# sharmaabhijith/safe-dreamer

Measured on AMD Instinct MI355X. Metric: imagined latent steps/sec at B16·L64·H15, 1/2/4/8 MI355X; WM-loss Δ vs ref, higher is better.
Workload: dtype f32 (split-bf16 gradient GEMMs); 1 GPU; dmc walker_walk vision 64x64x3, rep_loss=r2dreamer (BASELINE configs[1]), per-GPU B16 L64 H15; config=dmc/cnn, global_batch=16, per_gpu_batch=16, seq_len=64, imag_horizon=15, parallelism=dp1

## Files before the change

### safe-dreamer_amd/csrc/conv.hip

```cpp
#include <stdlib.h>

#include "gemm3_core.h"
#include "gemm6_core.h"
#include "gemm_core.h"
#include "sdhip.h"

extern "C" int sd_colsum(const float* in, float* out, int R, int N, long ld, int accumulate, sd_stream s);
extern "C" int sd_colsum_ws(const float* in, float* out, int R, int N, long ld, int accumulate, float* workspace,
                            sd_stream s);

namespace {
using namespace sdg;

struct Geom {
  const float* in;
  int Nb, Hs, Ws, C;
  int Hg, Wg;
  int kh, kw, pad, ups;
};

SD_DEV bool tap(const Geom& G, int n, int y, int x, int k, long& off) {
  const int t = k / G.C, c = k - t * G.C;
  const int ky = t / G.kw, kx = t - ky * G.kw;
  const int yy = y + ky - G.pad, xx = x + kx - G.pad;
// ... 439 lines not shown
                 : f32x4{0.f, 0.f, 0.f, 0.f};
    }
#pragma unroll
    for (int e = 0; e < NE; ++e) {
      const int i = tid + 256 * e;
      if (i < NEL) {
        const int c4 = i % CI4, pix = i / CI4;
        float h0, h1, h2, h3, m0, m1, m2, m3;
        const u32x2 h{bf16_pair(v[e][0], v[e][1], h0, h1), bf16_pair(v[e][2], v[e][3], h2, h3)};
        const float r0 = v[e][0] - h0, r1 = v[e][1] - h1, r2 = v[e][2] - h2, r3 = v[e][3] - h3;
        const u32x2 m{bf16_pair(r0, r1, m0, m1), bf16_pair(r2, r3, m2, m3)};
        const f32x4 l{r0 - m0, r1 - m1, r2 - m2, r3 - m3};
        __bf16* dst = patch6 + pix * CP + 4 * c4;
        *reinterpret_cast<u32x2*>(dst) = h;
        *reinterpret_cast<u32x2*>(dst + PLANE) = m;
        *reinterpret_cast<bf16x4*>(dst + 2 * PLANE) = __builtin_convertvector(l, bf16x4);
      }
    }
  }
  int pbase[2];
#pragma unroll
  for (int mt = 0; mt < 2; ++mt) {
    const int p = 32 * wave + 16 * mt + l16;
    pbase[mt] = ((p >> LW) * PW + (p & (W - 1))) * CP;
  }
  const __bf16* wl = wsp + (long)l16 * KP + 8 * q;
  bf16x8 b[2][TN][3];
  auto bload = [&](int kc, int s) {
#pragma unroll
    for (int j = 0; j < TN; ++j)
#pragma unroll
      for (int pl = 0; pl < 3; ++pl)
        b[s][j][pl] = *reinterpret_cast<const bf16x8*>(wl + ((long)pl * BN + 16 * j) * KP + 32 * kc);
  };
  f32x4 acc[2][TN];
#pragma unroll
  for (int i = 0; i < 2; ++i)
#pragma unroll
    for (int j = 0; j < TN; ++j) acc[i][j] = f32x4{0.f, 0.f, 0.f, 0.f};
  bload(0, 0);
  __syncthreads();
  auto chunk = [&](int kc, int s) {
    if (kc + 1 < NKC) bload(kc + 1, s ^ 1);
    int k0 = 32 * kc + 8 * q;
    k0 = k0 < K ? k0 : K - 8;
    const int tap = k0 / CI, c0 = k0 - tap * CI, ky = tap / KS, kx = tap - ky * KS;
    const int off = (ky * PW + kx) * CP + c0;
    bf16x8 a[2][3];
#pragma unroll
    for (int mt = 0; mt < 2; ++mt)
#pragma unroll
      for (int pl = 0; pl < 3; ++pl) a[mt][pl] = *reinterpret_cast<const bf16x8*>(patch6 + pl * PLANE + pbase[mt] + off);
#pragma unroll
    for (int mt = 0; mt < 2; ++mt)
#pragma unroll
      for (int j = 0; j < TN; ++j) {
        f32x4 c = acc[mt][j];
        c = __builtin_amdgcn_mfma_f32_16x16x32_bf16(a[mt][2], b[s][j][0], c, 0, 0, 0);
        c = __builtin_amdgcn_mfma_f32_16x16x32_bf16(a[mt][1], b[s][j][1], c, 0, 0, 0);
        c = __builtin_amdgcn_mfma_f32_16x16x32_bf16(a[mt][0], b[s][j][2], c, 0, 0, 0);
        c = __builtin_amdgcn_mfma_f32_16x16x32_bf16(a[mt][1], b[s][j][0], c, 0, 0, 0);
        c = __builtin_amdgcn_mfma_f32_16x16x32_bf16(a[mt][0], b[s][j][1], c, 0, 0, 0);
        acc[mt][j] = __builtin_amdgcn_mfma_f32_16x16x32_bf16(a[mt][0], b[s][j][0], c, 0, 0, 0);
      }
  };
  int kc = 0;
  for (; kc + 2 <= NKC; kc += 2) {
    chunk(kc, 0);
    chunk(kc + 1, 1);
  }
  if (kc < NKC) chunk(kc, 0);
  __syncthreads();
  pool_epilogue<BN, 32>(acc, reinterpret_cast<float*>(patch6), g, G, LW, lhw, bm0, nw, pooled, amax, y, rstd, eps,
                        nchw_flat);
}

template <int BN, int CI, int LW, int KS, int TPW, int MT = 2, int BROW = 40, class NW = const float*>
__global__ __launch_bounds__(512, 1) void conv_fwd6r_direct_pool(GemmArgs g, Geom G, int lhw,
                                                                  const __bf16* __restrict__ wsp, NW nw,
                                                                  float* pooled, uint8_t* amax, float* y, float* rstd,
                                                                  float eps, int nchw_flat) {
  constexpr int NTH = 512, TP = 16 * MT * (NTH / 64);
  constexpr int W = 1 << LW, R = TP / W, PH = R + KS - 1, PW = W + KS - 1, PAD = KS / 2;
  constexpr int NPIX = PH * PW, PLANE = NPIX * CI, K = KS * KS * CI, NKC = (K + 31) / 32, KP = NKC * 32, TN = BN / 16;
  constexpr int CI4 = CI / 4, NEL = PH * PW * CI4, NE = (NEL + NTH - 1) / NTH;
  constexpr int SB = 3 * BN * BROW, NPC = 3 * BN * 4, NPT = (NPC + NTH - 1) / NTH;
  auto poff = [](int pix, int c) { return ((c >> 3) * NPIX + pix) * 8 + (c & 7); };
  static_assert(CI % 8 == 0 && TP % W == 0 && BN % 16 == 0, "geometry");
  static_assert(TP * (BN + 1) * 4 <= 3 * PLANE * 2, "epilogue tile fits the patch area");
  typedef __bf16 bf16x8 __attribute__((ext_vector_type(8)));
  extern __shared__ __attribute__((aligned(16))) __bf16 patch6r[];
  const int tid = threadIdx.x, lane = tid & 63, wave = tid >> 6, l16 = lane & 15, q = lane >> 4;
  const int nwg = gridDim.x, ntiles = g.M / TP;
  const int wg = (nwg & 7) ? blockIdx.x : (blockIdx.x & 7) * (nwg >> 3) + (blockIdx.x >> 3);
  __bf16* bst = patch6r + 3 * PLANE;
  bf16x8 br[NPT];
  auto bload = [&](int kc) {
#pragma unroll
    for (int u = 0; u < NPT; ++u) {
      const int i = tid + NTH * u;
      if (i < NPC) br[u] = *reinterpret_cast<const bf16x8*>(wsp + (long)(i >> 2) * KP + 32 * kc + 8 * (i & 3));
    }
  };
  auto bstore = [&](int st) {
#pragma unroll
    for (int u = 0; u < NPT; ++u) {
      const int i = tid + NTH * u;
      if (i < NPC) *reinterpret_cast<bf16x8*>(bst + st * SB + (i >> 2) * BROW + 8 * (i & 3)) = br[u];
    }
  };
  f32x4 v[NE];
  auto load_patch = [&](int tile) {
    const int bm0 = tile * TP, n = bm0 >> lhw, y0 = (bm0 & ((1 << lhw) - 1)) >> LW;
#pragma unroll
    for (int e = 0; e < NE; ++e) {
      const int i = tid + NTH * e, c4 = i % CI4, pix = i / CI4, pc = pix % PW, pr = pix / PW;
      const int yy = y0 + pr - PAD, xx = pc - PAD;
      v[e] = (i < NEL && tile < ntiles && (unsigned)yy < (unsigned)G.Hs && (unsigned)xx < (unsigned)W)
                 ? *reinterpret_cast<const f32x4*>(G.in + (((long)n * G.Hs + yy) * W + xx) * CI + 4 * c4)
                 : f32x4{0.f, 0.f, 0.f, 0.f};
    }
  };
  auto store_patch = [&]() {
#pragma unroll
    for (int e = 0; e < NE; ++e) {
      const int i = tid + NTH * e;
      if (i < NEL) {
        const int c4 = i % CI4, pix = i / CI4;
        float h0, h1, h2, h3, m0, m1, m2, m3;
        const u32x2 h{bf16_pair(v[e][0], v[e][1], h0, h1), bf16_pair(v[e][2], v[e][3], h2, h3)};
        const float r0 = v[e][0] - h0, r1 = v[e][1] - h1, r2 = v[e][2] - h2, r3 = v[e][3] - h3;
        const u32x2 m{bf16_pair(r0, r1, m0, m1), bf16_pair(r2, r3, m2, m3)};
        const f32x4 l{r0 - m0, r1 - m1, r2 - m2, r3 - m3};
        __bf16* dst = patch6r + poff(pix, 4 * c4);
        *reinterpret_cast<u32x2*>(dst) = h;
        *reinterpret_cast<u32x2*>(dst + PLANE) = m;
        *reinterpret_cast<bf16x4*>(dst + 2 * PLANE) = __builtin_convertvector(l, bf16x4);
      }
    }
  };
  int pbase[MT];
#pragma unroll
  for (int mt = 0; mt < MT; ++mt) {
    const int p = 16 * MT * wave + 16 * mt + l16;
    pbase[mt] = (p >> LW) * PW + (p & (W - 1));
  }
  bload(0);
  load_patch(wg * TPW);
  for (int it = 0; it < TPW; ++it) {
  const int tile = wg * TPW + it;
  if (tile >= ntiles) break;
  if (it > 0) __syncthreads();
  store_patch();
  bstore(0);
  if (NKC > 1) bload(1);
  f32x4 acc[MT][TN];
#pragma unroll
  for (int i = 0; i < MT; ++i)
#pragma unroll
    for (int j = 0; j < TN; ++j) acc[i][j] = f32x4{0.f, 0.f, 0.f, 0.f};
  __syncthreads();
  if (it + 1 < TPW) load_patch(tile + 1);
  for (int kc = 0; kc < NKC; ++kc) {
    const __bf16* bs = bst + (kc & 1) * SB + l16 * BROW + 8 * q;
    bf16x8 b[TN][3];
#pragma unroll
    for (int j = 0; j < TN; ++j)
#pragma unroll
      for (int pl = 0; pl < 3; ++pl) b[j][pl] = *reinterpret_cast<const bf16x8*>(bs + (pl * BN + 16 * j) * BROW);
    int k0 = 32 * kc + 8 * q;
    k0 = k0 < K ? k0 : K - 8;
    const int tap = k0 / CI, c0 = k0 - tap * CI, ky = tap / KS, kx = tap - ky * KS;
    const int toff = ky * PW + kx;
    bf16x8 a[MT][3];
#pragma unroll
    for (int mt = 0; mt < MT; ++mt)
#pragma unroll
      for (int pl = 0; pl < 3; ++pl)
        a[mt][pl] = *reinterpret_cast<const bf16x8*>(patch6r + pl * PLANE + poff(pbase[mt] + toff, c0));
    if (kc + 1 < NKC) bstore((kc + 1) & 1);
    if (kc + 2 < NKC) bload(kc + 2);
#pragma unroll
    for (int mt = 0; mt < MT; ++mt)
#pragma unroll
      for (int j = 0; j < TN; ++j) {
        f32x4 c = acc[mt][j];
        c = __builtin_amdgcn_mfma_f32_16x16x32_bf16(a[mt][2], b[j][0], c, 0, 0, 0);
        c = __builtin_amdgcn_mfma_f32_16x16x32_bf16(a[mt][1], b[j][1], c, 0, 0, 0);
        c = __builtin_amdgcn_mfma_f32_16x16x32_bf16(a[mt][0], b[j][2], c, 0, 0, 0);
        c = __builtin_amdgcn_mfma_f32_16x16x32_bf16(a[mt][1], b[j][0], c, 0, 0, 0);
        c = __builtin_amdgcn_mfma_f32_16x16x32_bf16(a[mt][0], b[j][1], c, 0, 0, 0);
        acc[mt][j] = __builtin_amdgcn_mfma_f32_16x16x32_bf16(a[mt][0], b[j][0], c, 0, 0, 0);
      }
    __syncthreads();
  }
  if (it + 1 < TPW) bload(0);
  pool_epilogue<BN, 16 * MT>(acc, reinterpret_cast<float*>(patch6r), g, G, LW, lhw, tile * TP, nw, pooled, amax, y,
                             rstd, eps, nchw_flat);
  }
}

__global__ __launch_bounds__(256) void split3_weight(const float* __restrict__ w, __bf16* __restrict__ out, int rows,
                                                     int K, int KP) {
  const long i = (long)blockIdx.x * 256 + threadIdx.x;
  if (i >= (long)rows * KP) return;
  const int r = (int)(i / KP), k = (int)(i % KP);
  const float v = k < K ? w[(long)r * K + k] : 0.f;
  const __bf16 a0 = (__bf16)v;
  const float r1 = v - (float)a0;
  const __bf16 a1 = (__bf16)r1;
  const long pl = (long)rows * KP;
  out[i] = a0;
  out[pl + i] = a1;
  out[2 * pl + i] = (__bf16)(r1 - (float)a1);
}

template <int BN, int LW, int KS, int OCC, class NW = const float*>
__global__ __launch_bounds__(256, OCC) void conv_fwd_direct_pool_c4(GemmArgs g, Geom G, int lhw, int TPW,
                                                                    NW nw, float* pooled, uint8_t* amax,
                                                                    float* y, float* rstd, float eps, int nchw_flat) {
  constexpr int BM = 128, WM = 32, TM = WM / 16, TN = BN / 16, W = 1 << LW, R = BM / W;
  constexpr int PH = R + KS - 1, PW = W + KS - 1, PAD = KS / 2, NT = KS * KS;
  constexpr int NQ = PH * PW, NQT = (NQ + 255) / 256;
  float* smem = sd_smem<NQT * 256 * 4 + BM * (BN + 1)>();
  float* patch = smem;
  float* C = smem + NQT * 256 * 4;
  const int nwg = gridDim.x, ntiles = g.M / BM;
  const int wg = (nwg & 7) ? blockIdx.x : (blockIdx.x & 7) * (nwg >> 3) + (blockIdx.x >> 3);
  const int lane = threadIdx.x & 63, wave = threadIdx.x >> 6, l16 = lane & 15, q = lane >> 4;
  float bw[NT][TN];
  {
    const sd_rsrc rb = sd_make_rsrc(g.B, (long)g.N * g.ldb * 4);
#pragma unroll
    for (int t = 0; t < NT; ++t)
#pragma unroll
      for (int j = 0; j < TN; ++j) bw[t][j] = sd_bload1(rb, (uint32_t)(((16 * j + l16) * g.ldb + 4 * t + q) * 4));
  }
  EpiPre<BN> pre;
#pragma unroll
  for (int j = 0; j < TN; ++j) pre.bias[j] = g.bias ? g.bias[16 * j + l16] : 0.f;
#pragma unroll
  for (int k = 0; k < BN / 8; ++k) pre.nw[k] = nw_of(nw)[(threadIdx.x & 7) + 8 * k];
  const sd_rsrc rs = sd_make_rsrc(G.in, (long)G.Nb * G.Hs * G.Ws * 16);
  f32x4 v[NQT];
  auto load_patch = [&](int tile) {
    const int bm0 = tile * BM, n = bm0 >> lhw, y0 = (bm0 & ((1 << lhw) - 1)) >> LW;
#pragma unroll
    for (int u = 0; u < NQT; ++u) {
      const int i = threadIdx.x + 256 * u;
      const int py = i / PW, px = i % PW;
      const int yy = y0 + py - PAD, xx = px - PAD;
      const bool ok = i < NQ && tile < ntiles && (unsigned)yy < (unsigned)G.Hs && (unsigned)xx < (unsigned)W;
      v[u] = sd_bload4(rs, ok ? (uint32_t)(((n * G.Hs + yy) * W + xx) * 16) : SD_OOB);
    }
  };
  int abase[TM];
#pragma unroll
  for (int i = 0; i < TM; ++i) {
    const int p = wave * WM + 16 * i + l16;
    abase[i] = ((p >> LW) * PW + (p & (W - 1))) * 4 + q;
  }
  load_patch(wg * TPW);
  for (int it = 0; it < TPW; ++it) {
    const int tile = wg * TPW + it;
    if (tile >= ntiles) break;
#pragma unroll
    for (int u = 0; u < NQT; ++u) *reinterpret_cast<f32x4*>(patch + 4 * (threadIdx.x + 256 * u)) = v[u];
    __syncthreads();
    if (it + 1 < TPW) load_patch(tile + 1);
    f32x4 acc[TM][TN];
#pragma unroll
    for (int i = 0; i < TM; ++i)
#pragma unroll
      for (int j = 0; j < TN; ++j) acc[i][j] = f32x4{0.f, 0.f, 0.f, 0.f};
#pragma unroll
    for (int t = 0; t < NT; ++t) {
      const int toff = ((t / KS) * PW + t % KS) * 4;
      float a[TM];
#pragma unroll
      for (int i = 0; i < TM; ++i) a[i] = patch[abase[i] + toff];
#pragma unroll
      for (int i = 0; i < TM; ++i)
#pragma unroll
        for (int j = 0; j < TN; ++j)
          acc[i][j] = __builtin_amdgcn_mfma_f32_16x16x4f32(a[i], bw[t][j], acc[i][j], 0, 0, 0);
    }
    __syncthreads();
    pool_epilogue<BN, WM>(acc, C, g, G, LW, lhw, tile * BM, nw, pooled, amax, y, rstd, eps, nchw_flat, &pre);
  }
}


struct DirectW {
  const float* x;
  const float* dy;
  const uint8_t* amax;
  float* ws;
  int Nb, H, W, Ci, Co, kh, kw, pad, R, lw;
  int J, PW, PH, CP, DS, blocks;
};

constexpr int WD_VA = 4, WD_VP = 6;

template <int TM, bool PL>
struct WdF32 {
  const DirectW& d;
  const int tid, nA;
  float* const dyl;
  float* const xp;
  f32x4 ra[WD_VA];
  uint32_t aa[PL ? WD_VA : 1];
  SD_DEV WdF32(const DirectW& d_, float* lds, int tid_)
      : d(d_), tid(tid_), nA(d_.R * d_.W * d_.Co / 4), dyl(lds), xp(lds + d_.R * d_.W * d_.DS) {}
  SD_DEV void init() {
    for (int pix = tid; pix < d.PH * d.PW; pix += 512) {
      xp[pix * d.CP + d.Ci] = 1.f;
      xp[pix * d.CP + d.Ci + 1] = 0.f;
    }
  }
  SD_DEV void fetch_dy(int n, int y0) {
    const float* dsrc = d.dy + ((long)n * d.H + y0) * d.W * d.Co;
#pragma unroll
    for (int v = 0; v < WD_VA; ++v) {
      const int i = tid + 512 * v;
      if constexpr (PL) {
        ra[v] = f32x4{0.f, 0.f, 0.f, 0.f};
        aa[v] = 0xffffffffu;
        if (i < nA / 4) {
          const long pp = (((long)n * (d.H >> 1) + (y0 >> 1)) * (d.W >> 1)) * d.Co + 4 * i;
          ra[v] = *reinterpret_cast<const f32x4*>(d.dy + pp);
          aa[v] = *reinterpret_cast<const uint32_t*>(d.amax + pp);
        }
      } else {
        ra[v] = i < nA ? *reinterpret_cast<const f32x4*>(dsrc + 4 * i) : f32x4{0.f, 0.f, 0.f, 0.f};
      }
    }
  }
  SD_DEV void stage_dy() {
#pragma unroll
    for (int v = 0; v < WD_VA; ++v) {
      const int i = tid + 512 * v;
      if constexpr (PL) {
        if (i < nA / 4) {
          const int e = 4 * i, pl = e / d.Co, c = e - pl * d.Co;
          const int hw = d.W >> 1, pr = pl / hw, pc = pl - pr * hw;
#pragma unroll
          for (int qd = 0; qd < 4; ++qd) {
            const int p = (2 * pr + (qd >> 1)) * d.W + 2 * pc + (qd & 1);
            f32x4 val;
#pragma unroll
            for (int k = 0; k < 4; ++k) val[k] = ((aa[v] >> (8 * k)) & 0xffu) == (uint32_t)qd ? ra[v][k] : 0.f;
            *reinterpret_cast<f32x4*>(dyl + p * d.DS + c) = val;
          }
        }
      } else if (i < nA) {
        const int e = 4 * i, p = e / d.Co, c = e - p * d.Co;
        *reinterpret_cast<f32x4*>(dyl + p * d.DS + c) = ra[v];
      }
    }
  }
  SD_DEV void stage_patch(int pix, int c, const f32x4& v) { *reinterpret_cast<f32x4*>(xp + pix * d.CP + c) = v; }
  template <int NBW, bool WS>
  SD_DEV void contract(f32x4 (&acc)[TM][NBW], const int (&off)[NBW], int P, int wave, int l16, int q) {
    for (int s = WS ? wave : 0; s < P / 4; s += WS ? NW_D : 1) {
      const int p = 4 * s + q, py = p >> d.lw, px = p & (d.W - 1);
      float a[TM];
#pragma unroll
      for (int i = 0; i < TM; ++i) a[i] = dyl[p * d.DS + 16 * i + l16];
      const float* xb = xp + (py * d.PW + px) * d.CP;
      float bv[NBW];
#pragma unroll
      for (int b = 0; b < NBW; ++b) bv[b] = xb[off[b]];
#pragma unroll
      for (int b = 0; b < NBW; ++b)
#pragma unroll
        for (int i = 0; i < TM; ++i) acc[i][b] = __builtin_amdgcn_mfma_f32_16x16x4f32(a[i], bv[b], acc[i][b], 0, 0, 0);
    }
  }
};

SD_DEV uint32_t pack_split(float v) {
  const f32x4 x = {v, 0.f, 0.f, 0.f};
  sdb::bf16x4 hi, lo;
  sdb::split2(x, hi, lo);
  return (uint32_t)__builtin_bit_cast(uint16_t, hi[0]) | ((uint32_t)__builtin_bit_cast(uint16_t, lo[0]) << 16);
}

template <int TM, bool PL>
struct WdBf16x3 {
  typedef uint32_t u32x4 __attribute__((ext_vector_type(4)));
  const DirectW& d;
  const int tid;
  float* const xp;
  __bf16* const dyh;
  __bf16* const dyl;
  int nD, dq4, dc, dih, dsb;
  f32x4 rd[4];
  uint32_t aw[PL ? 4 : 1];
  int qd[PL ? 4 : 1];
  SD_DEV WdBf16x3(const DirectW& d_, float* lds, int tid_)
      : d(d_), tid(tid_), xp(lds), dyh(reinterpret_cast<__bf16*>(lds + d_.PH * d_.PW * d_.CP)),
        dyl(dyh + TM * 16 * d_.DS) {
    for (int e = tid; e < TM * 16 * d.DS; e += 512) {
      dyh[e] = (__bf16)0.f;
      dyl[e] = (__bf16)0.f;
    }
  }
  SD_DEV void init() {
    const int c4 = d.Co / 4, drest = tid / c4;
    nD = c4 * (d.R * d.W / 4);
    dq4 = tid % c4;
    dc = drest % 4, dih = (drest / 4) % 2, dsb = drest / 8;
    for (int pix = tid; pix < d.PH * d.PW; pix += 512) {
      reinterpret_cast<uint32_t*>(xp)[pix * d.CP + d.Ci] = pack_split(1.f);
      reinterpret_cast<uint32_t*>(xp)[pix * d.CP + d.Ci + 1] = 0u;
    }
  }
  SD_DEV void fetch_dy(int n, int y0) {
    [[maybe_unused]] const float* dsrc = d.dy + ((long)n * d.H + y0) * d.W * d.Co;
#pragma unroll
    for (int t = 0; t < 4; ++t) {
      const int px = 32 * dsb + dc + 4 * (4 * dih + t);
      if constexpr (PL) {
        const int yy = y0 + (px >> d.lw), xx = px & (d.W - 1);
        const long pp = (((long)n * (d.H >> 1) + (yy >> 1)) * (d.W >> 1) + (xx >> 1)) * d.Co + 4 * dq4;
        const bool ok = tid < nD;
        rd[t] = ok ? *reinterpret_cast<const f32x4*>(d.dy + pp) : f32x4{0.f, 0.f, 0.f, 0.f};
        aw[t] = ok ? *reinterpret_cast<const uint32_t*>(d.amax + pp) : 0xffffffffu;
        qd[t] = (yy & 1) * 2 + (xx & 1);
      } else {
        rd[t] = tid < nD ? *reinterpret_cast<const f32x4*>(dsrc + (long)px * d.Co + 4 * dq4)
                         : f32x4{0.f, 0.f, 0.f, 0.f};
      }
    }
  }
  SD_DEV void stage_dy() {
    if (tid < nD) {
      const int pos = 32 * dsb + 8 * dc + 4 * dih;
      if constexpr (PL) {
#pragma unroll
        for (int t = 0; t < 4; ++t)
#pragma unroll
          for (int k = 0; k < 4; ++k)
            if (((aw[t] >> (8 * k)) & 0xffu) != (uint32_t)qd[t]) rd[t][k] = 0.f;
      }
#pragma unroll
      for (int jj = 0; jj < 4; ++jj) {
        const f32x4 t = {rd[0][jj], rd[1][jj], rd[2][jj], rd[3][jj]};
        sdb::bf16x4 hi, lo;
        sdb::split2(t, hi, lo);
        const int o = (4 * dq4 + jj) * d.DS + pos;
        *reinterpret_cast<sdb::bf16x4*>(dyh + o) = hi;
        *reinterpret_cast<sdb::bf16x4*>(dyl + o) = lo;
      }
    }
  }
  SD_DEV void stage_patch(int pix, int c, const f32x4& v) {
    sdb::bf16x4 hi, lo;
    sdb::split2(v, hi, lo);
    const uint64_t h = __builtin_bit_cast(uint64_t, hi), l = __builtin_bit_cast(uint64_t, lo);
    u32x4 w;
#pragma unroll
    for (int k = 0; k < 4; ++k) w[k] = (uint32_t)((h >> (16 * k)) & 0xffffu) | ((uint32_t)((l >> (16 * k)) & 0xffffu) << 16);
    *reinterpret_cast<u32x4*>(xp + pix * d.CP + c) = w;
  }
  template <int NBW, bool WS>
  SD_DEV void contract(f32x4 (&acc)[TM][NBW], const int (&off)[NBW], int P, int wave, int l16, int q) {
    for (int s = WS ? wave : 0; s < P / 32; s += WS ? NW_D : 1) {
      sdb::bf16x8 ah[TM], al[TM];
#pragma unroll
      for (int i = 0; i < TM; ++i) {
        const int o = (16 * i + l16) * d.DS + 32 * s + 8 * q;
        ah[i] = *reinterpret_cast<const sdb::bf16x8*>(dyh + o);
        al[i] = *reinterpret_cast<const sdb::bf16x8*>(dyl + o);
      }
      int pb[8];
#pragma unroll
      for (int i = 0; i < 8; ++i) {
        const int p = 32 * s + 4 * i + q, py = p >> d.lw, px = p & (d.W - 1);
        pb[i] = (py * d.PW + px) * d.CP;
      }
#pragma unroll
      for (int b = 0; b < NBW; ++b) {
        const uint32_t* xu = reinterpret_cast<const uint32_t*>(xp);
        uint32_t wv[8];
#pragma unroll
        for (int i = 0; i < 8; ++i) wv[i] = xu[pb[i] + off[b]];
        u32x4 ph, pl;
#pragma unroll
        for (int i = 0; i < 4; ++i) {
          ph[i] = __builtin_amdgcn_perm(wv[2 * i + 1], wv[2 * i], 0x05040100u);
          pl[i] = __builtin_amdgcn_perm(wv[2 * i + 1], wv[2 * i], 0x07060302u);
        }
        const sdb::bf16x8 bh = __builtin_bit_cast(sdb::bf16x8, ph), bl = __builtin_bit_cast(sdb::bf16x8, pl);
#pragma unroll
        for (int i = 0; i < TM; ++i) {
          acc[i][b] = __builtin_amdgcn_mfma_f32_16x16x32_bf16(al[i], bh, acc[i][b], 0, 0, 0);
          acc[i][b] = __builtin_amdgcn_mfma_f32_16x16x32_bf16(ah[i], bl, acc[i][b], 0, 0, 0);
          acc[i][b] = __builtin_amdgcn_mfma_f32_16x16x32_bf16(ah[i], bh, acc[i][b], 0, 0, 0);
        }
      }
    }
  }
};

template <class M, int TM, int NBW, bool WS>
SD_DEV void wgrad_direct_body(const DirectW& d) {
  extern __shared__ __attribute__((aligned(16))) float lds[];
  const int tid = threadIdx.x, lane = tid & 63, wave = tid >> 6;
  const int l16 = lane & 15, q = lane >> 4;
  const int P = d.R * d.W;
  M m(d, lds, tid);
  int off[NBW];
#pragma unroll
  for (int b = 0; b < NBW; ++b) {
    const int j = 16 * (WS ? b : (blockIdx.x * NW_D + wave) * NBW + b) + l16;
    if (j < d.J) {
      const int t = j / d.Ci, ci = j - t * d.Ci, ky = t / d.kw, kx = t - ky * d.kw;
      off[b] = (ky * d.PW + kx) * d.CP + ci;
    } else {
      off[b] = d.Ci + (j == d.J ? 0 : 1);
    }
  }
  f32x4 acc[TM][NBW];
#pragma unroll
  for (int i = 0; i < TM; ++i)
#pragma unroll
    for (int b = 0; b < NBW; ++b) acc[i][b] = f32x4{0.f, 0.f, 0.f, 0.f};
  const int rows_per_img = d.H / d.R, cq = d.Ci / 4, nP = d.PH * d.PW * cq;
  f32x4 rp[WD_VP];
  auto fetch = [&](int rb) {
    const int n = rb / rows_per_img, y0 = (rb - n * rows_per_img) * d.R;
    m.fetch_dy(n, y0);
#pragma unroll
    for (int v = 0; v < WD_VP; ++v) {
      const int i = tid + 512 * v;
      f32x4 x = {0.f, 0.f, 0.f, 0.f};
      if (i < nP) {
        const int pix = i / cq, c = 4 * (i - pix * cq);
        const int py = pix / d.PW, px = pix - py * d.PW;
        const int iy = y0 - d.pad + py, ix = px - d.pad;
        if (iy >= 0 && iy < d.H && ix >= 0 && ix < d.W)
          x = *reinterpret_cast<const f32x4*>(d.x + (((long)n * d.H + iy) * d.W + ix) * d.Ci + c);
      }
      rp[v] = x;
    }
  };
  auto stage = [&]() {
    m.stage_dy();
#pragma unroll
    for (int v = 0; v < WD_VP; ++v) {
      const int i = tid + 512 * v;
      if (i < nP) {
        const int pix = i / cq, c = 4 * (i - pix * cq);
        m.stage_patch(pix, c, rp[v]);
      }
    }
  };
  m.init();
  int rb = blockIdx.y;
  if (rb < d.blocks) fetch(rb);
  for (; rb < d.blocks; rb += gridDim.y) {
    __syncthreads();
    stage();
    __syncthreads();
    if (rb + (int)gridDim.y < d.blocks) fetch(rb + gridDim.y);
    m.template contract<NBW, WS>(acc, off, P, wave, l16, q);
  }
  float* out = d.ws + (long)blockIdx.y * d.Co * (d.J + 1);
  if constexpr (WS) {
#pragma unroll
    for (int b = 0; b < NBW; ++b)
#pragma unroll
      for (int i = 0; i < TM; ++i) {
        __syncthreads();
#pragma unroll
        for (int r = 0; r < 4; ++r) lds[(wave * 4 + r) * 64 + lane] = acc[i][b][r];
        __syncthreads();
        if (tid < 256) {
          const int r = tid >> 6, ln = tid & 63;
          float v = 0.f;
#pragma unroll
          for (int w = 0; w < NW_D; ++w) v += lds[(w * 4 + r) * 64 + ln];
          const int j = 16 * b + (ln & 15), co = 16 * i + 4 * (ln >> 4) + r;
          if (j <= d.J && co < d.Co) out[(long)co * (d.J + 1) + j] = v;
        }
      }
    return;
  }
#pragma unroll
  for (int b = 0; b < NBW; ++b) {
    const int j = 16 * ((blockIdx.x * NW_D + wave) * NBW + b) + l16;
    if (j <= d.J) {
#pragma unroll
      for (int i = 0; i < TM; ++i)
#pragma unroll
        for (int r = 0; r < 4; ++r) {
          const int co = 16 * i + 4 * q + r;
          if (co < d.Co) out[(long)co * (d.J + 1) + j] = acc[i][b][r];
        }
    }
  }
}

template <int TM, int NBW, bool WS, bool PL = false>
__global__ __launch_bounds__(512) void conv_wgrad_direct(DirectW d) {
  wgrad_direct_body<WdF32<TM, PL>, TM, NBW, WS>(d);
}
template <int TM, int NBW, bool WS = false, bool PL = false>
__global__ __launch_bounds__(512) void conv_wgrad3_direct(DirectW d) {
  wgrad_direct_body<WdBf16x3<TM, PL>, TM, NBW, WS>(d);
}


template <class L, int ROWS>
struct KCSplit {
  L& l;
  SD_DEV explicit KCSplit(L& l_) : l(l_) {}
  SD_DEV void load(int k0, int kend) { l.load(k0, kend); }
  SD_DEV void store(__bf16* lds) const {
#pragma unroll
    for (int v = 0; v < L::NV; ++v) {
      const int i = threadIdx.x + v * 256;
      if ((v + 1) * 256 <= ROWS * BK / 4 || i < ROWS * BK / 4)
        sdb::split_store(lds + (i / (BK / 4)) * sdb::LROW + 4 * (i % (BK / 4)), l.st.r[v]);
    }
  }
};

template <int BN>
__global__ __launch_bounds__(256, 2) void conv_dgrad3(GemmArgs g, Geom G, int lw, int lhw) {
  __shared__ int tab[MAX_TAPQ];
  build_taps(tab, G, g.K);
  constexpr int BM = 128;
  const int bm0 = blockIdx.x * BM;
  Im2colRowsB<BM> la0(G, tab, g.M, bm0, lw, lhw);
  DenseKCB<BN> lb0(g.B, g.ldb, g.N, 0);
  KCSplit<Im2colRowsB<BM>, BM> la(la0);
  KCSplit<DenseKCB<BN>, BN> lb(lb0);
  f32x4 acc[2][BN / 16];
  sdb::gemm3_mainloop<BM, BN, 32, BN>(la, lb, 0, g.K, acc);
  epilogue16<BM, BN, 32, BN>(g, acc, bm0, 0, 0, 0);
}

template <int CIN, int NT, int LW, int KS, int NTHR>
__global__ __launch_bounds__(NTHR, 2) void conv_dgrad3_direct(const float* __restrict__ dout,
                                                               const __bf16* __restrict__ wsp, float* __restrict__ din,
                                                               int Nb, int H, int pad) {
  constexpr int MT = 4, TP = 16 * MT * (NTHR / 64);
  constexpr int W = 1 << LW, R = TP / W, PH = R + KS - 1, PW = W + KS - 1, NPIX = PH * PW;
  constexpr int PLANE = NPIX * CIN, K = KS * KS * CIN, NKC = (K + 31) / 32, KP = NKC * 32, NOUT = 16 * NT;
  constexpr int CIN4 = CIN / 4, NEL = PH * PW * CIN4, NE = (NEL + NTHR - 1) / NTHR;
  static_assert(CIN % 8 == 0 && R >= 1 && TP % W == 0, "geometry");
  auto poff = [](int pix, int c) { return ((c >> 3) * NPIX + pix) * 8 + (c & 7); };
  extern __shared__ __attribute__((aligned(16))) __bf16 patch[];
  const int tid = threadIdx.x, lane = tid & 63, wave = tid >> 6, l16 = lane & 15, q = lane >> 4;
  const int rows_per_img = H / R, n = blockIdx.x / rows_per_img, y0 = (blockIdx.x % rows_per_img) * R;
  {
    f32x4 v[NE];
#pragma unroll
    for (int e = 0; e < NE; ++e) {
      const int i = tid + NTHR * e, c4 = i % CIN4, pix = i / CIN4, pc = pix % PW, pr = pix / PW;
      const int y = y0 + pr - pad, x = pc - pad;
      v[e] = (i < NEL && y >= 0 && y < H && x >= 0 && x < W)
                 ? *reinterpret_cast<const f32x4*>(dout + (((long)n * H + y) * W + x) * CIN + 4 * c4)
                 : f32x4{0.f, 0.f, 0.f, 0.f};
    }
#pragma unroll
    for (int e = 0; e < NE; ++e) {
      const int i = tid + NTHR * e;
      if (i < NEL) {
        const int c4 = i % CIN4, pix = i / CIN4;
        sdb::bf16x4 hi, lo;
        sdb::split2(v[e], hi, lo);
        *reinterpret_cast<sdb::bf16x4*>(patch + poff(pix, 4 * c4)) = hi;
        *reinterpret_cast<sdb::bf16x4*>(patch + PLANE + poff(pix, 4 * c4)) = lo;
      }
    }
  }
  int pbase[MT];
#pragma unroll
  for (int mt = 0; mt < MT; ++mt) {
    const int p = 16 * MT * wave + 16 * mt + l16;
    pbase[mt] = (p >> LW) * PW + (p & (W - 1));
  }
  typedef __bf16 bf16x8 __attribute__((ext_vector_type(8)));
  constexpr int BROW = 40, SB = 2 * NOUT * BROW, NPC = 8 * NOUT, NPT = (NPC + NTHR - 1) / NTHR;
  __bf16* bst = patch + 2 * PLANE;
  bf16x8 br[NPT];
  auto bload = [&](int kc) {
#pragma unroll
    for (int u = 0; u < NPT; ++u) {
      const int i = tid + NTHR * u;
      if (i < NPC) br[u] = *reinterpret_cast<const bf16x8*>(wsp + (long)(i >> 2) * KP + 32 * kc + 8 * (i & 3));
    }
  };
  auto bstore = [&](int stage) {
#pragma unroll
    for (int u = 0; u < NPT; ++u) {
      const int i = tid + NTHR * u;
      if (i < NPC) *reinterpret_cast<bf16x8*>(bst + stage * SB + (i >> 2) * BROW + 8 * (i & 3)) = br[u];
    }
  };
  f32x4 acc[MT][NT];
#pragma unroll
  for (int i = 0; i < MT; ++i)
#pragma unroll
    for (int j = 0; j < NT; ++j) acc[i][j] = f32x4{0.f, 0.f, 0.f, 0.f};
  bload(0);
  bstore(0);
  if (NKC > 1) bload(1);
  __syncthreads();
  for (int kc = 0; kc < NKC; ++kc) {
    const __bf16* bs = bst + (kc & 1) * SB + l16 * BROW + 8 * q;
    bf16x8 bh[NT], bl[NT];
#pragma unroll
    for (int j = 0; j < NT; ++j) {
      bh[j] = *reinterpret_cast<const bf16x8*>(bs + 16 * j * BROW);
      bl[j] = *reinterpret_cast<const bf16x8*>(bs + (NOUT + 16 * j) * BROW);
    }
    int k0 = 32 * kc + 8 * q;
    k0 = k0 < K ? k0 : K - 8;
    const int tap = k0 / CIN, c0 = k0 - tap * CIN, ky = tap / KS, kx = tap - ky * KS;
    const int toff = ky * PW + kx;
    bf16x8 ah[MT], al[MT];
#pragma unroll
    for (int mt = 0; mt < MT; ++mt) {
      ah[mt] = *reinterpret_cast<const bf16x8*>(patch + poff(pbase[mt] + toff, c0));
      al[mt] = *reinterpret_cast<const bf16x8*>(patch + PLANE + poff(pbase[mt] + toff, c0));
    }
    if (kc + 1 < NKC) bstore((kc + 1) & 1);
    if (kc + 2 < NKC) bload(kc + 2);
#pragma unroll
    for (int mt = 0; mt < MT; ++mt)
#pragma unroll
      for (int j = 0; j < NT; ++j) {
        acc[mt][j] = __builtin_amdgcn_mfma_f32_16x16x32_bf16(al[mt], bh[j], acc[mt][j], 0, 0, 0);
        acc[mt][j] = __builtin_amdgcn_mfma_f32_16x16x32_bf16(ah[mt], bl[j], acc[mt][j], 0, 0, 0);
        acc[mt][j] = __builtin_amdgcn_mfma_f32_16x16x32_bf16(ah[mt], bh[j], acc[mt][j], 0, 0, 0);
      }
    __syncthreads();
  }
#pragma unroll
  for (int mt = 0; mt < MT; ++mt)
#pragma unroll
    for (int r = 0; r < 4; ++r) {
      const int p = 16 * MT * wave + 16 * mt + 4 * q + r, y = y0 + (p >> LW), x = p & (W - 1);
      float* o = din + (((long)n * H + y) * W + x) * NOUT + l16;
#pragma unroll
      for (int j = 0; j < NT; ++j) o[16 * j] = acc[mt][j][r];
    }
}

__global__ __launch_bounds__(256) void split_weight(const float* __restrict__ w, __bf16* __restrict__ out, int rows,
                                                    int K, int KP) {
  const long i = (long)blockIdx.x * 256 + threadIdx.x;
  if (i >= (long)rows * KP) return;
  const int r = (int)(i / KP), k = (int)(i % KP);
  const float v = k < K ? w[(long)r * K + k] : 0.f;
  const __bf16 hi = (__bf16)v;
  out[i] = hi;
  out[(long)rows * KP + i] = (__bf16)(v - (float)hi);
}

__global__ __launch_bounds__(256) void slab_reduce(const float* __restrict__ ws, int slabs, long n,
                                                   float* __restrict__ out, sd_wgrad_acc acc, int J, int cx) {
  __shared__ float part[4][64];
  const int lane = threadIdx.x & 63, wave = threadIdx.x >> 6;
  const long e = (long)blockIdx.x * 64 + lane;
  float v = 0.f;
  if (e < n) {
    int s = wave;
    for (; s + 12 < slabs; s += 16) {
      const float a0 = ws[(long)s * n + e], a1 = ws[(long)(s + 4) * n + e];
      const float a2 = ws[(long)(s + 8) * n + e], a3 = ws[(long)(s + 12) * n + e];
      v += (a0 + a1) + (a2 + a3);
    }
    for (; s < slabs; s += 4) v += ws[(long)s * n + e];
  }
  part[wave][lane] = v;
  __syncthreads();
  if (wave == 0 && e < n) {
    const float r = (part[0][lane] + part[1][lane]) + (part[2][lane] + part[3][lane]);
    if (!acc.dw) {
      out[e] = r;
    } else {
      const long co = e / (J + 1);
      const int j = (int)(e - co * (J + 1));
      if (j == J) {
        acc.db[co] += r;
      } else {
        const int tap = j / cx, c = j - tap * cx;
        if (c < acc.ci_w) acc.dw[(co * (J / cx) + tap) * acc.ci_w + c] += r;
      }
    }
  }
}

int ilog2_exact(int v) {
  if (v <= 0 || (v & (v - 1))) return -1;
  int l = 0;
  while ((1 << l) < v) ++l;
  return l;
}

template <int BM, int BN, int WM, int WN, bool VA, bool VB>
__global__ __launch_bounds__(256) void conv_fwd_kernel(GemmArgs g, Geom G) {
  const int bn0 = blockIdx.x * BN, bm0 = blockIdx.y * BM;
  Im2colRows<BM, VA> la(G, g.M, bm0);
  DenseOperand<BN, true, VB> lb(g.B, g.ldb, g.N, bn0);
  gemm_block<BM, BN, WM, WN>(g, la, lb, bm0, bn0, 0, 0, 0, g.K);
}

template <int BM, int BN, int WM, int WN, bool VA, bool VB>
__global__ __launch_bounds__(256) void conv_wgrad_kernel(GemmArgs g, Geom G, int J) {
  const int bn0 = blockIdx.x * BN, bm0 = blockIdx.y * BM;
  const int split = blockIdx.z;
  const int kbeg = split * g.kchunk;
  const int kend = min(g.K, kbeg + g.kchunk);
  DenseOperand<BM, false, VA> la(g.A, g.lda, g.M, bm0);
  Im2colCols<BN, VB> lb(G, J, bn0);
  gemm_block<BM, BN, WM, WN>(g, la, lb, bm0, bn0, 0, split, kbeg, kend);
}

template <int T, int VPT, class NW = const float* __restrict__>
__global__ void pool_rms_fwd(const float* __restrict__ x, NW w, float* __restrict__ pooled,
// ... 962 lines not shown
```

Baseline: 1.540 million imagined_latents/s.

## Split wgrad patch staging into hi/lo bf16 planes read via ds_read_tr16

The bf16x3 direct weight-gradient kernel now stores the im2col patch as two separate bf16 planes (hi and lo) instead of interleaved hi|lo 32-bit words. The B operand is loaded with the LDS transpose-read instruction ds_read_tr16_b64, so eight scalar LDS loads plus perm unpacking per column block become four transposed vector reads. Column offsets are recomputed per 4-lane group to match the transpose read pattern. This depends on the LDS layout and alignment lining up with the transpose-read semantics, and it changes how the bias/ones column is addressed.

```diff
diff --git a/safe-dreamer_amd/csrc/conv.hip b/safe-dreamer_amd/csrc/conv.hip
--- a/safe-dreamer_amd/csrc/conv.hip
+++ b/safe-dreamer_amd/csrc/conv.hip
@@ -765,6 +765,11 @@
 
 constexpr int WD_VA = 4, WD_VP = 6;
 
+SD_DEV int wd_tap_off(const DirectW& d, int j) {
+  const int t = j / d.Ci, ci = j - t * d.Ci, ky = t / d.kw, kx = t - ky * d.kw;
+  return (ky * d.PW + kx) * d.CP + ci;
+}
+
 template <int TM, bool PL>
 struct WdF32 {
   const DirectW& d;
@@ -781,6 +786,10 @@
       xp[pix * d.CP + d.Ci + 1] = 0.f;
     }
   }
+  SD_DEV int col_off(int j0, int l16) const {
+    const int j = j0 + l16;
+    return j < d.J ? wd_tap_off(d, j) : d.Ci + (j == d.J ? 0 : 1);
+  }
   SD_DEV void fetch_dy(int n, int y0) {
     const float* dsrc = d.dy + ((long)n * d.H + y0) * d.W * d.Co;
 #pragma unroll
@@ -842,19 +851,13 @@
   }
 };
 
-SD_DEV uint32_t pack_split(float v) {
-  const f32x4 x = {v, 0.f, 0.f, 0.f};
-  sdb::bf16x4 hi, lo;
-  sdb::split2(x, hi, lo);
-  return (uint32_t)__builtin_bit_cast(uint16_t, hi[0]) | ((uint32_t)__builtin_bit_cast(uint16_t, lo[0]) << 16);
-}
-
 template <int TM, bool PL>
 struct WdBf16x3 {
-  typedef uint32_t u32x4 __attribute__((ext_vector_type(4)));
+  typedef __attribute__((address_space(3))) sdb::bf16x4 lds_bf16x4;
   const DirectW& d;
   const int tid;
-  float* const xp;
+  __bf16* const xh;
+  __bf16* const xl;
   __bf16* const dyh;
   __bf16* const dyl;
   int nD, dq4, dc, dih, dsb;
@@ -862,8 +865,8 @@
   uint32_t aw[PL ? 4 : 1];
   int qd[PL ? 4 : 1];
   SD_DEV WdBf16x3(const DirectW& d_, float* lds, int tid_)
-      : d(d_), tid(tid_), xp(lds), dyh(reinterpret_cast<__bf16*>(lds + d_.PH * d_.PW * d_.CP)),
-        dyl(dyh + TM * 16 * d_.DS) {
+      : d(d_), tid(tid_), xh(reinterpret_cast<__bf16*>(lds)), xl(xh + d_.PH * d_.PW * d_.CP),
+        dyh(reinterpret_cast<__bf16*>(lds + d_.PH * d_.PW * d_.CP)), dyl(dyh + TM * 16 * d_.DS) {
     for (int e = tid; e < TM * 16 * d.DS; e += 512) {
       dyh[e] = (__bf16)0.f;
       dyl[e] = (__bf16)0.f;
@@ -874,10 +877,16 @@
     nD = c4 * (d.R * d.W / 4);
     dq4 = tid % c4;
     dc = drest % 4, dih = (drest / 4) % 2, dsb = drest / 8;
+    sdb::bf16x4 one, zero;
+    sdb::split2(f32x4{1.f, 0.f, 0.f, 0.f}, one, zero);
     for (int pix = tid; pix < d.PH * d.PW; pix += 512) {
-      reinterpret_cast<uint32_t*>(xp)[pix * d.CP + d.Ci] = pack_split(1.f);
-      reinterpret_cast<uint32_t*>(xp)[pix * d.CP + d.Ci + 1] = 0u;
-    }
+      *reinterpret_cast<sdb::bf16x4*>(xh + pix * d.CP + d.Ci) = one;
+      *reinterpret_cast<sdb::bf16x4*>(xl + pix * d.CP + d.Ci) = zero;
+    }
+  }
+  SD_DEV int col_off(int j0, int l16) const {
+    const int j = j0 + 4 * (l16 & 3);
+    return 2 * (j < d.J ? wd_tap_off(d, j) : d.Ci);
   }
   SD_DEV void fetch_dy(int n, int y0) {
     [[maybe_unused]] const float* dsrc = d.dy + ((long)n * d.H + y0) * d.W * d.Co;
@@ -921,15 +930,19 @@
   SD_DEV void stage_patch(int pix, int c, const f32x4& v) {
     sdb::bf16x4 hi, lo;
     sdb::split2(v, hi, lo);
-    const uint64_t h = __builtin_bit_cast(uint64_t, hi), l = __builtin_bit_cast(uint64_t, lo);
-    u32x4 w;
-#pragma unroll
-    for (int k = 0; k < 4; ++k) w[k] = (uint32_t)((h >> (16 * k)) & 0xffffu) | ((uint32_t)((l >> (16 * k)) & 0xffffu) << 16);
-    *reinterpret_cast<u32x4*>(xp + pix * d.CP + c) = w;
+    *reinterpret_cast<sdb::bf16x4*>(xh + pix * d.CP + c) = hi;
+    *reinterpret_cast<sdb::bf16x4*>(xl + pix * d.CP + c) = lo;
+  }
+  static SD_DEV sdb::bf16x8 tr_pair(uint32_t a0, uint32_t a1) {
+    const sdb::bf16x4 v0 = __builtin_amdgcn_ds_read_tr16_b64_v4bf16(reinterpret_cast<lds_bf16x4*>(a0));
+    const sdb::bf16x4 v1 = __builtin_amdgcn_ds_read_tr16_b64_v4bf16(reinterpret_cast<lds_bf16x4*>(a1));
+    return __builtin_shufflevector(v0, v1, 0, 1, 2, 3, 4, 5, 6, 7);
   }
   template <int NBW, bool WS>
   SD_DEV void contract(f32x4 (&acc)[TM][NBW], const int (&off)[NBW], int P, int wave, int l16, int q) {
-    for (int s = WS ? wave : 0; s < P / 32; s += WS ? NW_D : 1) {
+    const uint32_t xh0 = (uint32_t)reinterpret_cast<uintptr_t>(xh), plane = 2u * d.PH * d.PW * d.CP;
+    const int s0 = WS ? __builtin_amdgcn_readfirstlane(wave) : 0;
+    for (int s = s0; s < P / 32; s += WS ? NW_D : 1) {
       sdb::bf16x8 ah[TM], al[TM];
 #pragma unroll
       for (int i = 0; i < TM; ++i) {
@@ -937,25 +950,16 @@
         ah[i] = *reinterpret_cast<const sdb::bf16x8*>(dyh + o);
         al[i] = *reinterpret_cast<const sdb::bf16x8*>(dyl + o);
       }
-      int pb[8];
-#pragma unroll
-      for (int i = 0; i < 8; ++i) {
-        const int p = 32 * s + 4 * i + q, py = p >> d.lw, px = p & (d.W - 1);
-        pb[i] = (py * d.PW + px) * d.CP;
+      uint32_t pa[2];
+#pragma unroll
+      for (int r = 0; r < 2; ++r) {
+        const int p = 32 * s + 4 * ((l16 >> 2) + 4 * r) + q, py = p >> d.lw, px = p & (d.W - 1);
+        pa[r] = xh0 + 2u * ((py * d.PW + px) * d.CP);
       }
 #pragma unroll
       for (int b = 0; b < NBW; ++b) {
-        const uint32_t* xu = reinterpret_cast<const uint32_t*>(xp);
-        uint32_t wv[8];
-#pragma unroll
-        for (int i = 0; i < 8; ++i) wv[i] = xu[pb[i] + off[b]];
-        u32x4 ph, pl;
-#pragma unroll
-        for (int i = 0; i < 4; ++i) {
-          ph[i] = __builtin_amdgcn_perm(wv[2 * i + 1], wv[2 * i], 0x05040100u);
-          pl[i] = __builtin_amdgcn_perm(wv[2 * i + 1], wv[2 * i], 0x07060302u);
-        }
-        const sdb::bf16x8 bh = __builtin_bit_cast(sdb::bf16x8, ph), bl = __builtin_bit_cast(sdb::bf16x8, pl);
+        const sdb::bf16x8 bh = tr_pair(pa[0] + off[b], pa[1] + off[b]);
+        const sdb::bf16x8 bl = tr_pair(pa[0] + off[b] + plane, pa[1] + off[b] + plane);
 #pragma unroll
         for (int i = 0; i < TM; ++i) {
           acc[i][b] = __builtin_amdgcn_mfma_f32_16x16x32_bf16(al[i], bh, acc[i][b], 0, 0, 0);
@@ -976,15 +980,7 @@
   M m(d, lds, tid);
   int off[NBW];
 #pragma unroll
-  for (int b = 0; b < NBW; ++b) {
-    const int j = 16 * (WS ? b : (blockIdx.x * NW_D + wave) * NBW + b) + l16;
-    if (j < d.J) {
-      const int t = j / d.Ci, ci = j - t * d.Ci, ky = t / d.kw, kx = t - ky * d.kw;
-      off[b] = (ky * d.PW + kx) * d.CP + ci;
-    } else {
-      off[b] = d.Ci + (j == d.J ? 0 : 1);
-    }
-  }
+  for (int b = 0; b < NBW; ++b) off[b] = m.col_off(16 * (WS ? b : (blockIdx.x * NW_D + wave) * NBW + b), l16);
   f32x4 acc[TM][NBW];
 #pragma unroll
   for (int i = 0; i < TM; ++i)
```

New measurement: 1.560 million imagined_latents/s, median of 6. +1.2%, better.
